# kcleal/pywfa

Measured on AMD Instinct MI355X. Metric: pairwise alignments/sec, higher is better.
Workload: dtype int16x2 offsets (reads <= 512 bp), int32 results; 1 GPU; C2: 10000000 x 150bp pairs/GPU, 2% error, gap-affine 0/4/6/2, end-to-end, scope=score, 2-bit reads resident in HBM; pairs_per_gpu=10000000, read_length=150, parallelism=pairs sharded over 1 GPU(s), no collective

## Files before the change

### pywfa_amd/csrc/host_core.hpp

```cpp
#pragma once
#include <hip/hip_runtime.h>
#include <stdarg.h>
#include <stddef.h>
#include <stdint.h>
#include <stdio.h>
#include <stdlib.h>
#include <string.h>
#include <limits.h>
#include <sched.h>
#include <string>
#include <map>
#include <unordered_map>
#include <vector>
#include <algorithm>
#include <thread>
#include <memory>
#include <atomic>

#include "wfa_hip.h"
#include "wfa_common.hpp"
#include "wfa_band.hpp"

namespace wfa { struct WfaPieceDesc; }

#pragma GCC visibility push(hidden)

extern thread_local std::string g_error;

#define WFA_COUNTER_WORDS 256
#define WFA_KNOBS(F)                                                                                              \
  F(ARENA_KB) F(BAND_DEBUG) F(BAND_SLIM) F(BAND_LDS_MAX) F(BAND_NO_WIN) F(BAND_SPLIT_MIN) F(NO_TINY_INLINE) F(BILEVEL) F(BILEVEL_WIDE_LEVELS) F(BILEVEL_PER_CU) F(BILEVEL_I32) F(BILEVEL_QCAP) F(BILEVEL_LEVELS) F(BILEVEL_LDS) F(BILEVEL_NO_1024) F(BILEVEL_HUGE_MIN) F(BILEVEL_LDS_W) F(BILEVEL_NO_SEQL) F(LANE_DYN) F(LANE_DYN_WAVES) F(BAND_LEFTOVER_WAVES_PER_CU) F(BAND_NCH) F(BAND_NO_LDS) F(BAND_NO_SPLIT) F(BAND_PB) F(PIPE_TAIL) F(LEN16) F(MAILBOX) F(MAILBOX_IDLE_US) F(TILE32)     \
  F(BAND_RECORDS) F(BAND_SPLIT_ROUNDS) F(BAND_WAVES_PER_CU) F(NO_BAND) F(NO_FAST) F(NO_SEGFULL) F(SEGFULL_PAIRS)     \
  F(SEGFULL_STAGES) F(STAGE_TIMING) F(LANE_HEUR32) F(THREADS) F(TINY_BATCH) F(WAVES_PER_CU) F(FAST_WAVES_PER_CU) F(TIMING)          \
  F(LANE_FULL) F(LANE_FULL_SPLIT) F(LANE_HEUR) F(SEG_HEUR) F(LANE_LDS_PAD_KB) F(LANE_MIN_PAIRS) F(PIPE_CHUNK) F(PIPE_THREADS) F(PACK_THREADS) F(NO_TINY_BAND) F(NO_TINY_POLL) F(UP_STREAMS) F(NO_DUAL) F(NO_WIDE) F(WIDE_ADAPT) F(WIDE_GROWS) F(WIDE_LDS_KB) F(WIDE_THREADS) F(TILE) F(TILE_T) F(TILE_WT) F(TILE_THREADS) F(TILE_PER_CU) F(NO_PIPE) F(HOST_PACK) F(GENERAL_PB) F(LANE_WAVES_PER_CU) F(LANE_REFILL_MIN) F(LANE_WINFIN) F(LANE_DEBUG) F(NO_TINY) F(PILOT_PCT) F(WIDE_ADAPT_LDS) F(LANE_NARROW_WAVES) F(PILOT_NARROW_PCT) F(CROSS_BAND) F(CROSS_TOPK_CHUNK) F(REDUCE_TIMING)
enum WfaKnob {
#define WFA_KNOB_ENUM(n) K_##n,
  WFA_KNOBS(WFA_KNOB_ENUM)
#undef WFA_KNOB_ENUM
  K_COUNT
};
struct WfaKnobs {
  int value[K_COUNT];
  bool set[K_COUNT];
  std::string fast_stages;
  void load() {
    static const char* const names[K_COUNT] = {
#define WFA_KNOB_NAME(n) "WFA_HIP_" #n,
        WFA_KNOBS(WFA_KNOB_NAME)
#undef WFA_KNOB_NAME
// ... 81 lines not shown
  std::vector<wfa::WfaPieceDesc> h_pieces;
  uint32_t* d_len16 = nullptr;
  wfa::WfaPieceDesc* d_pieces = nullptr;
  int max_width = 0;
  int max_len = 0;
  int64_t packed_bytes = 0;
  int64_t ops_bytes = 0;
  uint8_t* d_bytes = nullptr;
  int64_t* d_pboff = nullptr;
  int64_t* d_tboff = nullptr;
  WfaPairMeta* d_meta = nullptr;
  uint32_t* d_words = nullptr;
  uint8_t* d_flags = nullptr;
  int32_t* d_score = nullptr;
  int32_t* d_status = nullptr;
  uint8_t* d_ops = nullptr;
  int64_t* d_cigar_off = nullptr;
  int64_t* d_cigar_begin = nullptr;
  int32_t* d_cigar_len = nullptr;
  uint32_t* d_list_packed = nullptr;
  uint32_t* d_list_bytes = nullptr;
  uint32_t n_packed = 0, n_bytes = 0;
  uint32_t* d_fb_list2[2] = {nullptr, nullptr};
  const uint32_t* leftover_count = nullptr;
  uint32_t* d_ovf_list[2] = {nullptr, nullptr};
  uint32_t* d_counters = nullptr;
  std::vector<hipEvent_t> ev;
  size_t ev_used = 0;
  int runs_pending = 0;
  double ms_sum = 0.0; int ms_runs = 0;
// ... 122 lines not shown
```

### pywfa_amd/csrc/wfa_common.hpp

```cpp
#pragma once
#include "wfa_rtc_compat.hpp"

#define WFA_OFFSET_NULL (-1073741824)

#define WFA_INTERNAL_FALLBACK  (-1000)
#define WFA_INTERNAL_OVERFLOW  (-1001)

struct WfaPairMeta {
  uint32_t p_woff;
  uint32_t t_woff;
  int32_t plen;
  int32_t tlen;
};

struct WfaDevConfig {
  int32_t metric;
  int32_t match;
  int32_t x, o1, e1, o2, e2;
  int32_t scope;
  int32_t endsfree;
  int32_t pbf, pef, tbf, tef;
  int32_t heuristic;
  int32_t min_wf_len, max_dist_thr, steps_between, xdrop;
  int32_t max_steps;
// ... 53 lines not shown
  int g;
  int32_t* hist;
  long long hist_stride;
  int4* end_state;
  uint32_t work_begin;
  uint2* codes;
  int codes_cap;
  int ef, pbf, pef, tbf, tef;
  int heur, min_wf_len, max_dist_thr, steps_between;
  int max_steps;
  int xdrop;
  uint32_t* dyn_next;
  uint32_t dyn_chunk;
  int lin;
  int scope;
};

template <int W>
__device__ __forceinline__ int seg_from_below(int v) {
  if (W <= 16) {
    int r = __builtin_amdgcn_update_dpp(WFA_OFFSET_NULL, v, 0x111 , 0xf, 0xf, false);
    if (W == 8 && (threadIdx.x & 7) == 0) r = WFA_OFFSET_NULL;
    return r;
  }
  int r = __builtin_amdgcn_update_dpp(WFA_OFFSET_NULL, v, 0x138 , 0xf, 0xf, false);
  if (W == 32 && (threadIdx.x & 31) == 0) r = WFA_OFFSET_NULL;
  return r;
}
template <int W>
__device__ __forceinline__ int seg_from_above(int v) {
  if (W <= 16) {
// ... 13 lines not shown
```

### pywfa_amd/csrc/wfa_hip.hip

```cpp
#include <hip/hip_runtime.h>
#include <stdint.h>
#include <stdio.h>
#include <stdlib.h>
#include <string.h>
#include <limits.h>
#include <string>
#include <map>
#include <unordered_map>
#include <vector>
#include <algorithm>
#include <chrono>
#include <thread>
#include <memory>
#include <atomic>
#include <mutex>
#include <functional>
#include <ctype.h>
#include <pthread.h>
#include <sched.h>
#include <unistd.h>
#include <sys/syscall.h>

#include "host_core.hpp"
#include "wfa_pack.hpp"
// ... 306 lines not shown
  return WFA_HIP_OK;
}

extern "C" const char* wfa_hip_last_error(const wfa_hip_aligner_t* al) { return al ? al->err.c_str() : g_error.c_str(); }

wfa_hip_batch* batch_new(wfa_hip_aligner* al) {
  wfa_hip_batch* b = new wfa_hip_batch();
  b->al = al;
  al->live_batches += 1;
  return b;
}

void batch_free(wfa_hip_batch* b) {
  if (!b) return;
  (void)hipSetDevice(b->al->device);
  void* ptrs[] = {b->d_bytes, b->d_pboff, b->d_tboff, b->d_meta, b->d_words, b->d_flags, b->d_score, b->d_status,
                  b->d_ops, b->d_cigar_off, b->d_cigar_begin, b->d_cigar_len, b->d_list_packed, b->d_list_bytes,
                  b->d_fb_list2[0], b->d_fb_list2[1], b->d_ovf_list[0], b->d_ovf_list[1], b->d_counters,
                  b->d_plen, b->d_tlen, b->d_run_count, b->d_locs, b->d_run_off, b->d_len16, b->d_pieces};
  const bool timing = b->al->knobs.set[K_TIMING];
  const double t0 = timing ? std::chrono::duration<double, std::milli>(std::chrono::steady_clock::now().time_since_epoch()).count() : 0.0;
  if (b->ran && !b->synced && b->last_stream) (void)hipStreamSynchronize(b->last_stream);
  (void)hipStreamSynchronize(b->al->stream);
  const double t1 = timing ? std::chrono::duration<double, std::milli>(std::chrono::steady_clock::now().time_since_epoch()).count() : 0.0;
  for (void* p : ptrs) pool_release(b->al, p);
  for (hipEvent_t e : b->ev) (void)hipEventDestroy(e);
  if (b->upload_event) (void)hipEventDestroy(b->upload_event);
  const double t2 = timing ? std::chrono::duration<double, std::milli>(std::chrono::steady_clock::now().time_since_epoch()).count() : 0.0;
  wfa_hip_aligner* al = b->al;
  delete b;
  if (timing) fprintf(stderr, "[wfa_hip] batch_free: sync %.3f ms, release %.3f ms, host free %.3f ms\n", t1 - t0, t2 - t1,
// ... 326 lines not shown
  return WFA_HIP_OK;
}

bool wildcard_in_acgt(int wc) {
  return wc == 'A' || wc == 'C' || wc == 'G' || wc == 'T' || wc == 'a' || wc == 'c' || wc == 'g' || wc == 't';
}

int batch_alloc_common(wfa_hip_aligner* al, wfa_hip_batch* b, uint64_t total_words, int zero_tail) {
  const int64_t n = b->n;
  const size_t nn = (size_t)std::max<int64_t>(n, 1);
  HIP_TRY(al, pool_alloc(al, (void**)&b->d_meta, nn * sizeof(WfaPairMeta)));
  HIP_TRY(al, pool_alloc(al, (void**)&b->d_words, (size_t)total_words * sizeof(uint32_t)));
  HIP_TRY(al, pool_alloc(al, (void**)&b->d_flags, nn));
  HIP_TRY(al, pool_alloc(al, (void**)&b->d_score, nn * sizeof(int32_t)));
  HIP_TRY(al, pool_alloc(al, (void**)&b->d_status, nn * sizeof(int32_t)));
  HIP_TRY(al, pool_alloc(al, (void**)&b->d_fb_list2[0], nn * sizeof(uint32_t)));
  HIP_TRY(al, pool_alloc(al, (void**)&b->d_fb_list2[1], nn * sizeof(uint32_t)));
  HIP_TRY(al, pool_alloc(al, (void**)&b->d_counters, WFA_COUNTER_WORDS * sizeof(uint32_t)));
  HIP_TRY(al, hipMemsetAsync(b->d_counters, 0, WFA_COUNTER_WORDS * sizeof(uint32_t), al->stream));
  HIP_TRY(al, hipMemsetAsync(b->d_flags, 0, nn, al->stream));
  HIP_TRY(al, hipMemsetAsync(b->d_words + (total_words - (uint64_t)zero_tail), 0, (size_t)zero_tail * sizeof(uint32_t), al->stream));
  if (b->cfg.scope == WFA_SCOPE_FULL) {
    HIP_TRY(al, pool_alloc(al, (void**)&b->d_ops, (size_t)std::max<int64_t>(b->ops_bytes, 1)));
    HIP_TRY(al, pool_alloc(al, (void**)&b->d_cigar_off, ((size_t)n + 1) * sizeof(int64_t)));
    HIP_TRY(al, pool_alloc(al, (void**)&b->d_cigar_begin, nn * sizeof(int64_t)));
    HIP_TRY(al, pool_alloc(al, (void**)&b->d_cigar_len, nn * sizeof(int32_t)));
    HIP_TRY(al, pool_alloc(al, (void**)&b->d_ovf_list[0], nn * sizeof(uint32_t)));
    HIP_TRY(al, pool_alloc(al, (void**)&b->d_ovf_list[1], nn * sizeof(uint32_t)));
    HIP_TRY(al, hipMemcpyAsync(b->d_cigar_off, b->h_coff.data(), ((size_t)n + 1) * sizeof(int64_t), hipMemcpyHostToDevice, al->stream));
  }
// ... 1430 lines not shown
  if (!stages_env && b->stage_pick != 0 && c.in_count == nullptr) {
    stages = (b->stage_pick == 16) ? (b->narrow_pick == 1 ? "0189" : "189") : (b->stage_pick == 32) ? "89" : "9";
  }
  int variants[6] = {-1, -1, -1, -1, -1, -1};
  int nv = 0;
  for (const char* c = stages; *c && nv < 6; ++c) {
    const int v = *c - '0';
    if (v < 0 || v > 9) continue;
    if (v <= 1) {
      if (p.shape == WFA_SHAPE_RTC && (v == 0 || !p.lane_shape_fits)) continue;
    }
    variants[nv++] = v;
  }
  if (nv == 0) variants[nv++] = 6;
  int lane_passes = 0;
  for (int pass = 0; pass < nv; ++pass) {
    uint32_t* out_list = c.out_list(b);
    uint32_t* out_count = c.next_count(b);
    StageTimer timer(al, stream);
    int lrc;
    if (variants[pass] <= 1) {
      const bool narrow = variants[pass] == 0;
      const int lane_k = lane_passes++;
      uint32_t lane_dyn = (c.in_n >= 65536u && lane_k < 2) ? (uint32_t)std::max(0, knob(al, K_LANE_DYN, 192)) : 0u;
      const int dyn_waves = narrow ? knob(al, K_LANE_NARROW_WAVES, 24) : knob(al, K_LANE_DYN_WAVES, 16);
      if (lane_dyn && c.in_count != nullptr) {
        const int64_t expect = (b->narrow_permille >= 0 && variants[0] == 0) ? (int64_t)c.in_n * b->narrow_permille / 1000 : 0;
        const int64_t per_wave = expect / std::max<int64_t>(1, (int64_t)al->cu_count * dyn_waves * 2);
        lane_dyn = (uint32_t)std::max<int64_t>(64, std::min<int64_t>(lane_dyn, per_wave));
      }
      lrc = wfa::launch_lane(p.shape, p.sh, al->cu_count,
                             lane_dyn ? dyn_waves : knob(al, K_LANE_WAVES_PER_CU, 48),
                             wfa::lane_refill_arg(knob(al, K_LANE_REFILL_MIN, 8), knob(al, K_LANE_WINFIN, 1) != 0), b->max_len, stream, b->d_words, b->d_meta,
                             c.in_list, c.in_count, c.in_n, b->d_score, b->d_status, out_list, out_count,
                             (knob(al, K_LANE_DEBUG, 0) && al->ws) ? al->ws : nullptr, knob(al, K_LANE_LDS_PAD_KB, 0), knob(al, K_LANE_MIN_PAIRS, 0),
                             b->d_counters + (lane_k == 0 ? CNT_LANE_DYN0 : CNT_LANE_DYN1), lane_dyn, narrow ? 4 : 8);
      if (knob(al, K_LANE_DEBUG, 0) && al->ws) {
        unsigned long long c[10] = {0, 0, 0, 0, 0, 0, 0, 0, 0, 0};
        hipStreamSynchronize(stream); hipMemcpy(c, al->ws, sizeof(c), hipMemcpyDeviceToHost); hipMemset(al->ws, 0, sizeof(c));
        fprintf(stderr, "[wfa_hip] lane kernel: %llu wave-steps, %llu refills, %llu parked runs, %llu parked rounds, %llu probe blocks, %llu second-run rounds, "
                        "%llu hand-over blocks, %llu second runs, %llu entries, %llu entry rounds\n", c[0], c[1], c[2], c[3], c[4], c[5], c[6], c[7], c[8], c[9]);
      }
    } else {
      lrc = wfa::launch_seg(b->dcfg, al->cu_count, knob(al, K_FAST_WAVES_PER_CU, 256), stream, b->d_words, b->d_meta, c.in_list, c.in_count,
                            c.in_n, b->d_score, b->d_status, out_list, out_count, variants[pass]);
    }
    if (lrc != 0) { al->err = "fast kernel launch failed"; return WFA_HIP_EDEVICE; }
    if (timer.on) {
      uint32_t handed = 0;
      const float ms = timer.stop(out_count, &handed);
      fprintf(stderr, "[wfa_hip] stage %d (variant %d): %.3f ms, handed on %u pairs\n", pass, variants[pass], ms, handed);
    }
    c.advance(b, out_list, out_count);
  }
  return WFA_HIP_OK;
}

static int run_laneh_stage(wfa_hip_aligner* al, wfa_hip_batch* b, hipStream_t stream, const CascadePlan& p, Chain& c) {
  uint32_t* out_list = c.out_list(b);
  uint32_t* out_count = c.next_count(b);
// ... 1077 lines not shown
```

### pywfa_amd/csrc/wfa_lane.hpp

```cpp
#pragma once
#include "wfa_rtc_compat.hpp"
#include "wfa_common.hpp"
#include "wfa_hip.h"
#ifndef __HIPCC_RTC__
#include "wfa_rtc.hpp"
#include "wfa_shapes.hpp"
#endif

namespace wfa {

typedef short lane_s2 __attribute__((ext_vector_type(2)));
typedef unsigned short lane_u2 __attribute__((ext_vector_type(2)));

#define WFA_LANE_NULL16 (-16384)
#define WFA_LANE_NULL2 0xC000C000u
#ifndef WFA_LANE_DEBUG_COUNTERS
#define WFA_LANE_DEBUG_COUNTERS 0
#endif
#ifndef WFA_LANE_REGION_MARKS
#define WFA_LANE_REGION_MARKS 0
#endif
#if WFA_LANE_REGION_MARKS
#define WFA_LANE_MARK(name) asm volatile("; WFA_MARK " name ::: "memory")
#else
// ... 58 lines not shown
wfa_lane_kernel(const FastArgs a, const int slot_words_seq, const int refill_arg) {
  static_assert(!(FULL && HEUR), "the general form is score only");
  static_assert(NRP == 8 || (HEUR && NRP == 16) || (NRP == 4 && !FULL && !HEUR && LIN == 0),
                "the wider band exists in the general form only, the narrow one in the plain score-only form only");
  const int refill_min = refill_arg & 0xff;
  constexpr int NR = NRP, W = 2 * NR, H = NR;
  constexpr int DM = (X > OE) ? X : OE;
  constexpr int NEVER = 0x7fffffff;
  constexpr bool ENTRY = !FULL && !HEUR && LIN == 0;
  constexpr int K = ENTRY ? OE : 0, NCH = (OE + X - 1) / X;
  constexpr bool WINCH = ENTRY && NCH <= 2;
  constexpr uint32_t LNM = WINCH ? 0x3ffu : 0xffffu;
  constexpr int MH = (2 * OE) / X;
  static_assert(NCH - 1 <= MH && MH * X <= 2 * OE, "the chain's own end cells lie within the Hamming bound");
  const int mh = (refill_arg & 0x100) ? MH : NCH - 1;
  constexpr int NREC = LaneFull<OE, E>::NREC;
  extern __shared__ uint32_t lds[];
  const int slot_words = slot_words_seq;
  const int lane = threadIdx.x;
  uint32_t nwork = __builtin_amdgcn_readfirstlane(a.nwork_dev ? *a.nwork_dev : a.nwork);
  const bool dyn = !FULL && a.dyn_next != nullptr;
  bool exhausted = !dyn;
  uint32_t begin, end;
  auto grab = [&](uint32_t& b_, uint32_t& e_) -> bool {
    uint32_t nb = 0;
    if (lane == 0) nb = atomicAdd(a.dyn_next, a.dyn_chunk);
    nb = __builtin_amdgcn_readfirstlane(nb);
    if (nb >= nwork) return false;
    b_ = nb; e_ = (uint32_t)min((unsigned long long)nwork, (unsigned long long)nb + a.dyn_chunk);
    return true;
  };
  if (dyn) {
    if (!grab(begin, end)) return;
  } else {
    const uint32_t per = __builtin_amdgcn_readfirstlane((nwork + gridDim.x - 1) / gridDim.x);
    const unsigned long long begin64 = (unsigned long long)blockIdx.x * per;
    if (begin64 >= nwork) return;
    begin = (uint32_t)begin64;
    end = (uint32_t)min((unsigned long long)nwork, begin64 + per);
  }

  uint32_t pid0, pw0, ln0, pid1, pw1, ln1;
  __shared__ short wch[(WINCH && NCH == 2) ? 128 : 1];
  auto window_chain = [&](uint32_t wb, uint32_t& pid, uint32_t& pw, uint32_t& ln) -> uint32_t {
    WFA_LANE_MARK("entry_begin");
    WFA_LANE_COUNT(8);
    const int pl = (int)(ln & 0xffffu), tl = (int)(ln >> 16);
    const int nwp = (pl + 15) >> 4, ntot = nwp + ((tl + 15) >> 4), ak = tl - pl, L = min(pl, tl);
    const bool inw = (unsigned long long)wb + lane < end;
    const bool elig = inw && !(ln == 0xffffffffu || ntot + 1 > slot_words_seq || ak < 1 - 2 * H || ak > 2 * H - 1);
    bool act = elig;
    bool hact = elig && ak == 0, hend = false;
    int hm = 0;
    const uint32_t* pp = a.words + pw;
    int ch[NCH];
#pragma unroll
    for (int c = 0; c < NCH; ++c) ch[c] = WFA_LANE_NULL16;
    int ci = 0;
    const int imax = slot_words_seq >> 1;
    int base = 0;
#pragma nounroll
    for (int i = 0; i < imax && __any(act || hact); i += 2) {
      WFA_LANE_MARK("entryround_begin");
      WFA_LANE_COUNT(9);
      uint32_t x0 = 0u, x1 = 0u;
      const bool on = act || hact;
      if (on && base < L) x0 = pp[0] ^ pp[nwp];
      if (on && base + 16 < L) x1 = pp[1] ^ pp[nwp + 1];
      const int nb = L - base;
      const uint32_t k0 = nb >= 16 ? 0x55555555u : nb > 0 ? (0x55555555u >> (32 - 2 * nb)) : 0u;
      const uint32_t k1 = nb >= 32 ? 0x55555555u : nb > 16 ? (0x55555555u >> (64 - 2 * nb)) : 0u;
      unsigned long long d = (unsigned long long)((x0 | (x0 >> 1)) & k0) | ((unsigned long long)((x1 | (x1 >> 1)) & k1) << 32);
// ... 11 lines not shown
      const bool last = base + 32 >= L;
      const bool endc = act && last;
#pragma unroll
      for (int k = 0; k < NCH; ++k) ch[k] = (endc && ci == k) ? L : ch[k];
      act = act && !endc;
      hend = hend || (hact && last);
      hact = hact && !last && hm <= mh;
      pp += 2; base += 32;
      WFA_LANE_MARK("entryround_end");
    }
    const bool fin = hend && hm <= mh;
    if (fin) {
      a.score[pid] = -__mul24(hm * X, a.g);
      a.status[pid] = 0;
    }
    const uint32_t c0 = (uint32_t)ch[0];
    uint32_t lnc = elig ? (ln | ((c0 & 0x3fu) << 10) | ((c0 >> 6) << 26)) : ln;
    const bool keep = inw && !fin;
    const unsigned long long km = __ballot(keep);
    int dst = lane;
    if (__ballot(fin)) {
      const int rk = (int)__builtin_amdgcn_mbcnt_hi((uint32_t)(km >> 32), __builtin_amdgcn_mbcnt_lo((uint32_t)km, 0u));
      dst = keep ? rk : (int)__builtin_popcountll(km) + lane - rk;
      pid = (uint32_t)__builtin_amdgcn_ds_permute(dst << 2, (int)pid);
      pw = (uint32_t)__builtin_amdgcn_ds_permute(dst << 2, (int)pw);
      lnc = (uint32_t)__builtin_amdgcn_ds_permute(dst << 2, (int)lnc);
    }
    if constexpr (NCH == 2) wch[64 + dst] = (short)ch[1];
    ln = lnc;
    WFA_LANE_MARK("entry_end");
    return (uint32_t)__builtin_popcountll(km);
  };
  auto load_window = [&](uint32_t wb, uint32_t& pid, uint32_t& pw, uint32_t& ln) {
    const unsigned long long idx = (unsigned long long)wb + lane;
    pid = 0u; pw = 0u; ln = 0u;
    if (idx < end) {
      pid = a.worklist ? a.worklist[a.work_begin + idx] : (uint32_t)(a.work_begin + idx);
      const WfaPairMeta m = a.meta[pid];
      pw = m.p_woff;
      ln = (m.plen > WFA_FAST_MAX_LEN || m.tlen > WFA_FAST_MAX_LEN) ? 0xffffffffu : ((uint32_t)m.plen | ((uint32_t)m.tlen << 16));
    }
  };
  uint32_t wbase = begin, next_i = begin;
  uint32_t wn0 = 0u, wp0 = 0u, wn1 = 0u, wnext = begin;
  bool wmeta = false;
  auto slice_done = [&]() -> bool {
    if constexpr (WINCH) return wp0 >= wn0 && wn1 == 0u && wnext >= end;
    else return next_i >= end;
  };
  if constexpr (!WINCH) {
    load_window(wbase, pid0, pw0, ln0);
    load_window(wbase + 64u, pid1, pw1, ln1);
  } else {
    pid0 = pw0 = ln0 = pid1 = pw1 = ln1 = 0u;
  }

// ... 38 lines not shown
    WFA_LANE_MARK("looptop_begin");
    const int nidle = __builtin_popcountll(idle);
    if (!exhausted && slice_done() && (nidle >= refill_min || idle == ~0ull)) {
      if (grab(begin, end)) {
        wbase = begin; next_i = begin;
        if constexpr (WINCH) { wn0 = wp0 = wn1 = 0u; wnext = begin; wmeta = false; }
        else { load_window(wbase, pid0, pw0, ln0); load_window(wbase + 64u, pid1, pw1, ln1); }
      } else exhausted = true;
    }
    if (!slice_done() && (nidle >= refill_min || idle == ~0ull)) {
      WFA_LANE_MARK("refill_begin");
      WFA_LANE_COUNT(1);
      if constexpr (WINCH) {
#pragma nounroll
        while (wn1 == 0u && wnext < end) {
          if (!wmeta) load_window(wnext, pid1, pw1, ln1);
          wmeta = false;
          wn1 = window_chain(wnext, pid1, pw1, ln1);
          wnext = (end - wnext > 64u) ? wnext + 64u : end;
          if (wp0 >= wn0) {
            pid0 = pid1; pw0 = pw1; ln0 = ln1;
            if constexpr (NCH == 2) wch[lane] = wch[64 + lane];
            wn0 = wn1; wp0 = 0u; wn1 = 0u;
          }
        }
      }
      const bool is_idle = __builtin_amdgcn_inverse_ballot_w64(idle);
      const uint32_t rank = __builtin_amdgcn_mbcnt_hi((uint32_t)(idle >> 32), __builtin_amdgcn_mbcnt_lo((uint32_t)idle, 0u));
      const uint32_t navail = WINCH ? (wn0 - wp0) + wn1 : end - next_i;
      const bool take = is_idle && rank < navail;
      const uint32_t src = WINCH ? wp0 + rank : next_i + rank - wbase;
      const bool hi_w = src >= (WINCH ? wn0 : 64u);
      const int sl = (int)((WINCH ? (hi_w ? src - wn0 : src) : src) & 63u);
// ... 142 lines not shown
              if constexpr (!WINCH) { if (fin) lim[r] = WFA_LANE_NULL2; }
            }
            if constexpr (!WINCH) { if (fin) { deadline = NEVER; jt = 0; tend = 0xffffu; } }
          }
        }
      }
      if constexpr (WINCH) {
        __builtin_amdgcn_s_waitcnt(0x0F70);
        asm volatile("" ::: "memory");
      }
      if constexpr (WINCH) {
        if (wp0 >= wn0) {
          pid0 = pid1; pw0 = pw1; ln0 = ln1;
          if constexpr (NCH == 2) wch[lane] = wch[64 + lane];
          wp0 -= wn0; wn0 = wn1; wn1 = 0u;
          if (wnext < end) { load_window(wnext, pid1, pw1, ln1); wmeta = true; }
        }
      } else if (next_i - wbase >= 64u) {
        pid0 = pid1; pw0 = pw1; ln0 = ln1; wbase += 64u;
        load_window(wbase + 64u, pid1, pw1, ln1);
      }
      WFA_LANE_MARK("refill_end");
      if (WINCH && ntake == 0u && idle == ~0ull) continue;
    } else if (idle == ~0ull && exhausted) {
      rej_flush();
      break;
    }

    int hot_j = -1, hot_x = 0, hot_left = 0;
#pragma unroll
    for (int r = 0; r < NR; ++r) {
// ... 280 lines not shown
  else if (heur) hipLaunchKernelGGL((wfa_lane_kernel<X, OE, E, false, true>), dim3(grid), dim3(64), smem, stream, a, slot_words, refill_min);
  else if (full) hipLaunchKernelGGL((wfa_lane_kernel<X, OE, E, true>), dim3(grid), dim3(64), smem, stream, a, slot_words, refill_min);
  else hipLaunchKernelGGL((wfa_lane_kernel<X, OE, E, false>), dim3(grid), dim3(64), smem, stream, a, slot_words, refill_min);
  return hipGetLastError() == hipSuccess ? 0 : -1;
}

inline bool lane_heur_config(const WfaDevConfig& c, int ncomp) {
  return ncomp == 3 && c.match == 0 && c.wildcard < 0 && (c.heuristic == 0 || c.heuristic == 1);
}

inline int lane_slot_words(int max_len) {
  const int w = 2 * ((max_len + 15) >> 4) + 1;
  return w | 1;
}

inline int lane_refill_arg(int refill_min, bool winfin) { return (refill_min & 0xff) | (winfin ? 0x100 : 0); }

inline int lane_full_records(int OE, int E) { return 2 * (OE - E) + E * 17 + 1; }
inline void lane_full_geometry(uint32_t nwork, int cu_count, int per_cu, int min_pairs, int OE, int E, long long* grid_out, int* cap_out) {
  if (min_pairs <= 0) min_pairs = 256;
  long long grid = (long long)cu_count * per_cu;
  const long long max_grid = ((long long)nwork + min_pairs - 1) / std::max(min_pairs, 64);
  if (grid > max_grid) grid = max_grid;
  if (grid < 1) grid = 1;
  const long long per = ((long long)nwork + grid - 1) / grid;
  const int nrec = lane_full_records(OE, E);
  *grid_out = grid;
  *cap_out = (int)(per * nrec / 32 + 2 * nrec + 8);
}

#define WFA_LANE_RUN_SLOT 32
// ... 17 lines not shown
  if (a.lin) shape_idx = WFA_SHAPE_RTC;
  if (nrp != 8 && nrp != 4) return -1;
  if (nrp == 4 && (shape_idx == WFA_SHAPE_RTC || full || heur)) return -1;
  if (shape_idx == WFA_SHAPE_RTC) {
    struct { FastArgs a; int slot_words; int refill_min; } args = {a, slot_words, refill_min};
    return rtc_launch("wfa_lane.hpp", lane_rtc_name(sh, full, heur, a.lin), (unsigned)grid, 64, smem, stream, &args, sizeof(args));
  }
  return with_shape_index<affine_shape_count>(shape_idx, [&](auto i) {
    return launch_lane_unit<decltype(i)::value>((unsigned)grid, smem, stream, a, slot_words, refill_min, full, heur, nrp);
  });
}

inline int launch_lane(int shape_idx, const PenaltyShape& sh, int cu_count, int per_cu, int refill_min, int max_len, hipStream_t stream, const uint32_t* words,
                       const WfaPairMeta* meta, const uint32_t* worklist, const uint32_t* nwork_dev, uint32_t nwork,
                       int32_t* score, int32_t* status, uint32_t* fb_list, uint32_t* fb_count, int32_t* debug_counters = nullptr, int lds_pad_kb = 0,
                       int min_pairs = 0, uint32_t* dyn_next = nullptr, uint32_t dyn_chunk = 0, int nrp = 8) {
  FastArgs a = FastArgs();
  a.dyn_next = dyn_chunk ? dyn_next : nullptr; a.dyn_chunk = dyn_chunk;
  a.words = words; a.meta = meta; a.worklist = worklist; a.nwork_dev = nwork_dev; a.nwork = nwork;
  a.score = score; a.status = status; a.fb_list = fb_list; a.fb_count = fb_count;
  a.g = sh.g;
  a.hist = debug_counters; a.hist_stride = 0; a.end_state = nullptr; a.work_begin = 0;
  a.ef = a.pbf = a.pef = a.tbf = a.tef = 0; a.heur = 0; a.min_wf_len = a.max_dist_thr = a.steps_between = 0; a.max_steps = INT_MAX;
  return launch_lane_args(shape_idx, sh, cu_count, per_cu, refill_min, max_len, stream, a, false, lds_pad_kb, min_pairs, 0, nrp);
}

#endif

}
```

### pywfa_amd/csrc/wfa_seg.hpp

```cpp
#pragma once
#include "wfa_rtc_compat.hpp"
#include "wfa_common.hpp"
#include "wfa_hip.h"
#ifndef __HIPCC_RTC__
#include <string>
#include "wfa_rtc.hpp"
#include "wfa_shapes.hpp"
#endif

namespace wfa {

__device__ __forceinline__ uint32_t ffbl_u32(uint32_t x) {
  uint32_t r;
  asm("v_ffbl_b32 %0, %1" : "=v"(r) : "v"(x));
  return r;
}

template <int W>
__device__ __forceinline__ int seg_min(int v) {
  static_assert(W == 8 || W == 16 || W == 32, "segments inside a 32-lane group");
  v = min(v, __builtin_amdgcn_update_dpp(v, v, 0xB1 , 0xf, 0xf, false));
  v = min(v, __builtin_amdgcn_update_dpp(v, v, 0x4E , 0xf, 0xf, false));
  v = min(v, __builtin_amdgcn_update_dpp(v, v, 0x141 , 0xf, 0xf, false));
  if (W >= 16) v = min(v, __builtin_amdgcn_update_dpp(v, v, 0x140 , 0xf, 0xf, false));
// ... 3 lines not shown
template <int W>
__device__ __forceinline__ int seg_max(int v) { return ~seg_min<W>(~v); }

template <int X, int OE, int E, int W, bool LAZY, bool FULL, bool HEUR = false, int LIN = 0>
__global__ void __launch_bounds__(64)
wfa_seg_kernel(const FastArgs a) {
  static_assert(!(LAZY && FULL), "the history of a step is stored in the step itself");
  static_assert(!HEUR || (!LAZY && !FULL && W <= 32), "the general form: score only, every cell extended in its own step");
  static_assert(!LAZY || (X >= 2 && OE >= 2), "the lazy extension needs a wavefront to be consumed two steps after it is made (M is read at lags X and OE)");
  static_assert(W == 8 || W == 16 || W == 32 || W == 64, "segment width");
  constexpr int DM = (X > OE) ? X : OE;
  constexpr int NS = 64 / W, H = W / 2, LW = (W == 64) ? 6 : (W == 32) ? 5 : (W == 16) ? 4 : 3;
  constexpr unsigned long long FIELD = (W == 64) ? ~0ull : ((1ull << (W & 63)) - 1ull);
  constexpr int SW = WFA_FAST_WORDS;
  constexpr int NEVER = 0x7fffffff;
  __shared__ uint32_t lds[NS * 2 * SW + 4];
  __shared__ uint32_t ring[2][64];
  __shared__ uint32_t fbuf[64];
  __shared__ uint32_t rpid[64];
  __shared__ int rscore[64];
  const int lane = threadIdx.x;
  const int seg = lane >> LW;
  const int l = lane & (W - 1);
  const int pbias = seg * 2 * SW * 16, tbias = pbias + SW * 16;
  int kb = pbias - (l - H);
  uint32_t nwork = __builtin_amdgcn_readfirstlane(a.nwork_dev ? *a.nwork_dev : a.nwork);
  if (FULL && a.nwork_dev) {
    const uint32_t cap = a.nwork;
    if (nwork > cap) {
      for (uint32_t i = cap + blockIdx.x * 64u + threadIdx.x; i < nwork + 63u; i += gridDim.x * 64u) {
// ... 7 lines not shown
          a.fb_list[slot + __builtin_amdgcn_mbcnt_hi((uint32_t)(bm >> 32), __builtin_amdgcn_mbcnt_lo((uint32_t)bm, 0u))] = pid;
          a.status[pid] = WFA_INTERNAL_FALLBACK;
        }
      }
      nwork = cap;
    }
  }
  const uint32_t per = __builtin_amdgcn_readfirstlane((nwork + gridDim.x - 1) / gridDim.x);
  const unsigned long long begin64 = (unsigned long long)blockIdx.x * per;
  if (begin64 >= nwork) return;
  const uint32_t begin = (uint32_t)begin64;
  const uint32_t end = (uint32_t)min((unsigned long long)nwork, begin64 + per);

  uint32_t pid0, pid1;
  WfaPairMeta m0, m1;
  auto load_window = [&](uint32_t wb, uint32_t& pid, WfaPairMeta& m) {
    const unsigned long long idx = (unsigned long long)wb + lane;
    pid = 0u; m.p_woff = 0u; m.t_woff = 0u; m.plen = 0; m.tlen = 0;
    if (idx < end) { pid = a.worklist ? a.worklist[a.work_begin + idx] : (uint32_t)(a.work_begin + idx); m = a.meta[pid]; }
  };
  uint32_t wbase = begin;
  load_window(wbase, pid0, m0);
  load_window(wbase + 64u, pid1, m1);
  auto prefetch = [&](uint32_t i, uint32_t slot) {
    if (i < end) {
      const int r = (int)(i - wbase);
      uint32_t pw; int pl, tl;
      if (r < 64) {
        pw = __builtin_amdgcn_readlane(m0.p_woff, r);
        pl = __builtin_amdgcn_readlane(m0.plen, r); tl = __builtin_amdgcn_readlane(m0.tlen, r);
      } else {
        pw = __builtin_amdgcn_readlane(m1.p_woff, r - 64);
        pl = __builtin_amdgcn_readlane(m1.plen, r - 64); tl = __builtin_amdgcn_readlane(m1.tlen, r - 64);
      }
      const int ntot = ((pl + 15) >> 4) + ((tl + 15) >> 4);
      if (lane < ntot) __builtin_amdgcn_global_load_lds(a.words + pw + lane, &ring[slot][0], 4, 0, 0);
    }
  };
// ... 38 lines not shown
  int last_nonnull = 0, unreach_t = NEVER;
  bool edge = false;
  uint32_t want = (1u << NS) - 1u;
  uint32_t busy = 0;
  int gstep = 0;
  unsigned long long mcur = 0ull, mold = 0ull;

  while (true) {
    if (want) {
      do {
        const int s = __builtin_ctz(want);
        want &= want - 1u;
        if (next_i < end) {
          const uint32_t i = next_i++;
          const int r = (int)(i - wbase);
          int pl, tl; uint32_t pid;
          if (r < 64) {
            pl = __builtin_amdgcn_readlane(m0.plen, r); tl = __builtin_amdgcn_readlane(m0.tlen, r);
            pid = __builtin_amdgcn_readlane(pid0, r);
          } else {
            pl = __builtin_amdgcn_readlane(m1.plen, r - 64); tl = __builtin_amdgcn_readlane(m1.tlen, r - 64);
            pid = __builtin_amdgcn_readlane(pid1, r - 64);
          }
          const int pbf_ = (HEUR && a.ef) ? a.pbf : 0, tbf_ = (HEUR && a.ef) ? a.tbf : 0;
          const int dlo = min(-pbf_, tl - pl), dhi = max(tbf_, tl - pl);
          const bool bad = pl > WFA_FAST_MAX_LEN || tl > WFA_FAST_MAX_LEN ||
                           (HEUR ? (dhi - dlo > W - 3 || pbf_ > pl || tbf_ > tl) : (tl - pl < 1 - 2 * H || tl - pl > 2 * H - 1));
          const int akk = bad ? 0x7fff : tl - pl;
          const int c = bad ? 0 : (HEUR ? ((dlo + dhi + 1) >> 1) : ((tl - pl + 1) >> 1));
          const int nwp = (pl + 15) >> 4, ntot = nwp + ((tl + 15) >> 4);
          if (i + 1u < end) __builtin_amdgcn_s_waitcnt(0xF71);
          else __builtin_amdgcn_s_waitcnt(0xF70);
          uint32_t w = ring[par][lane];
          asm volatile("" : "+v"(w));
          if (!bad && lane < ntot) lds[s * 2 * SW + lane + ((lane >= nwp) ? SW - nwp : 0)] = w;
          prefetch(i + 2u, par);
          par ^= 1u;
          if (seg == s) {
            const int k = l - H + c;
            kb = pbias - k;
            target = (k == akk) ? tl : NEVER;
            lim = min(tl, pl + k);
            spair = pid; s0 = gstep;
            deadline = bad ? gstep - 1
                           : HEUR ? gstep + 4 * (pl + tl) + 64
                           : gstep + min(2 * (OE - E) + E * (2 * c + 2 * H - akk), 2 * (OE - E) + E * (2 * H + 2 - 2 * c + akk)) + (LAZY ? 1 : 0)
                                   - (FULL ? 1 : 0);
            if (FULL) { tslot = i; hp = reinterpret_cast<uint8_t*>(a.hist + (long long)i * a.hist_stride) + (k & (W - 1)); code = 0; }
            cur = (bad || k != 0) ? WFA_OFFSET_NULL : 0;
            if (HEUR) {
              if (!bad && a.ef && k >= -pbf_ && k <= tbf_) cur = max(k, 0);
              if (a.ef) target = bad ? NEVER : min(max(tl, pl + k - a.pef), max(pl + k, tl - a.tef));
              hdl = max(tl, pl + k); hjt = akk - (c - H); hdinit = max(pl, tl); steps_wait = a.steps_between; edge = false; have_max_sw = false;
              last_nonnull = 0; unreach_t = NEVER;
            }
#pragma unroll
            for (int d = 0; d < DM; ++d) Mh[d] = WFA_OFFSET_NULL;
#pragma unroll
            for (int d = 0; d < E; ++d) { Ih[d] = WFA_OFFSET_NULL; Dh[d] = WFA_OFFSET_NULL; }
          }
          if (LAZY) {
            const unsigned long long sm = FIELD << (s * W);
            mold &= ~sm;
            mcur = (mcur & ~sm) | (bad ? 0ull : (1ull << (s * W + H - c)));
          }
          busy |= 1u << s;
        }
      } while (want);
      if (!busy) break;
    }
    if (!LAZY) {
      int left = (cur >= 0) ? lim - cur : 0;
      if (__any(left > 0)) {
        int h = max(cur, 0) + tbias, v = max(cur + kb, pbias);
        bool more;
        do {
          const int pi = v >> 4, ti = h >> 4;
          const uint32_t p0 = lds[pi], p1 = lds[pi + 1], p2 = lds[pi + 2];
          const uint32_t t0 = lds[ti], t1 = lds[ti + 1], t2 = lds[ti + 2];
// ... 159 lines not shown
      int nm = max(nd, max(mx + 1, ni));
      if (nm > lim) nm = WFA_OFFSET_NULL;
#pragma unroll
      for (int d = E - 1; d > 0; --d) { Ih[d] = Ih[d - 1]; Dh[d] = Dh[d - 1]; }
      Ih[0] = ni; Dh[0] = nd;
      cur = nm;
      if (LAZY) { mold = mcur; mcur = __ballot(nm >= 0); }
      if (HEUR) {
        const unsigned long long eb = __ballot((l == 0 || l == W - 1) && (nm & ni & nd) >= 0);
        edge = ((eb >> (seg * W)) & FIELD) != 0ull;
      }
    }
    ++gstep;
    if (next_i - wbase >= 64u) {
      pid0 = pid1; m0 = m1; wbase += 64u;
      load_window(wbase + 64u, pid1, m1);
    }
  }
  res_flush();
  fb_flush();
}

#ifndef __HIPCC_RTC__
template <int I> int launch_seg_unit(int w, bool lazy, unsigned grid, hipStream_t stream, const FastArgs& a);
template <int I> int launch_seg_full_unit(int w, unsigned grid, hipStream_t stream, const FastArgs& a);
template <int I> int launch_seg_heur_unit(unsigned grid, hipStream_t stream, const FastArgs& a);

inline int seg_shape(const WfaDevConfig& c, PenaltyShape* sh) {
  *sh = penalty_shape(c, false);
  const int i = builtin_shape(*sh);
  if (i >= 0 && !(c.rtc && rtc_force_all())) return i;
// ... 83 lines not shown
inline void seg_full_slot(const WfaDevConfig& c, int w, int max_len, long long* code_ints, long long* event_ints, long long* slot_ints);
inline int seg_full_records(const WfaDevConfig& c, int w) {
  PenaltyShape sh;
  if (seg_shape(c, &sh) < 0) return 0;
  return 2 * (sh.OE - sh.E) + sh.E * (w + 1) + 3;
}

inline void seg_full_slot(const WfaDevConfig& c, int w, int max_len, long long* code_ints, long long* event_ints, long long* slot_ints) {
  *code_ints = (((long long)seg_full_records(c, w) * w + 15) & ~15ll) / 4;
  *event_ints = ((2ll * max_len + 16 + 15) & ~15ll) / 4;
  *slot_ints = (*code_ints + *event_ints + 2ll * max_len + 8 + 15) & ~15ll;
}

inline int launch_seg(const WfaDevConfig& c, int cu_count, int per_cu, hipStream_t stream, const uint32_t* words,
                      const WfaPairMeta* meta, const uint32_t* worklist, const uint32_t* nwork_dev, uint32_t nwork,
                      int32_t* score, int32_t* status, uint32_t* fb_list, uint32_t* fb_count, int variant) {
  FastArgs a = FastArgs();
  a.words = words; a.meta = meta; a.worklist = worklist; a.nwork_dev = nwork_dev; a.nwork = nwork;
  a.score = score; a.status = status; a.fb_list = fb_list; a.fb_count = fb_count;
  a.hist = nullptr; a.hist_stride = 0; a.end_state = nullptr; a.work_begin = 0;
  PenaltyShape sh;
  const int idx = seg_shape(c, &sh);
  if (idx < 0) return -1;
  a.g = sh.g;
  long long grid = (long long)cu_count * per_cu;
  if (!nwork_dev && grid > (long long)nwork) grid = nwork;
  if (grid < 1) grid = 1;
  const bool lazy = variant >= 6;
  const int w = (variant == 3 || variant == 7) ? 8 : (variant == 4 || variant == 8) ? 32 : (variant == 5 || variant == 9) ? 64 : 16;
  if (idx == WFA_SHAPE_RTC) return launch_seg_rtc(sh, w, lazy, false, false, (unsigned)grid, stream, a);
  return with_shape_index<affine_shape_count>(idx, [&](auto i) { return launch_seg_unit<decltype(i)::value>(w, lazy, (unsigned)grid, stream, a); });
}
// ... 5 lines not shown
```

Before: 4.369 billion alignments/s.

## Carry lane-kernel entry wavefront state into later passes to skip recomputation

The first lane pass now writes each eligible pair's early match-chain offsets, packed as two int16 values, into a new per-pair entry buffer. Later lane passes and the segmented fallback kernel read this buffer and resume the wavefront at score K instead of restarting at zero, skipping the opening steps for pairs passed on from earlier passes. This costs an extra 4-byte global store per pair and a load per retried pair, plus more complex initialisation logic in the seg kernel. That logic could be wrong in edge cases, such as equal-length pairs whose chain already reaches the end. It is enabled by default for non-full scopes and shapes with at most two chain entries.

Result: no change. 4.410 billion alignments/s (median of 6 runs) (+0.9%).

```diff
diff --git a/pywfa_amd/csrc/host_core.hpp b/pywfa_amd/csrc/host_core.hpp
--- a/pywfa_amd/csrc/host_core.hpp
+++ b/pywfa_amd/csrc/host_core.hpp
@@ -32,7 +32,7 @@
   F(ARENA_KB) F(BAND_DEBUG) F(BAND_SLIM) F(BAND_LDS_MAX) F(BAND_NO_WIN) F(BAND_SPLIT_MIN) F(NO_TINY_INLINE) F(BILEVEL) F(BILEVEL_WIDE_LEVELS) F(BILEVEL_PER_CU) F(BILEVEL_I32) F(BILEVEL_QCAP) F(BILEVEL_LEVELS) F(BILEVEL_LDS) F(BILEVEL_NO_1024) F(BILEVEL_HUGE_MIN) F(BILEVEL_LDS_W) F(BILEVEL_NO_SEQL) F(LANE_DYN) F(LANE_DYN_WAVES) F(BAND_LEFTOVER_WAVES_PER_CU) F(BAND_NCH) F(BAND_NO_LDS) F(BAND_NO_SPLIT) F(BAND_PB) F(PIPE_TAIL) F(LEN16) F(MAILBOX) F(MAILBOX_IDLE_US) F(TILE32)     \
   F(BAND_RECORDS) F(BAND_SPLIT_ROUNDS) F(BAND_WAVES_PER_CU) F(NO_BAND) F(NO_FAST) F(NO_SEGFULL) F(SEGFULL_PAIRS)     \
   F(SEGFULL_STAGES) F(STAGE_TIMING) F(LANE_HEUR32) F(THREADS) F(TINY_BATCH) F(WAVES_PER_CU) F(FAST_WAVES_PER_CU) F(TIMING)          \
-  F(LANE_FULL) F(LANE_FULL_SPLIT) F(LANE_HEUR) F(SEG_HEUR) F(LANE_LDS_PAD_KB) F(LANE_MIN_PAIRS) F(PIPE_CHUNK) F(PIPE_THREADS) F(PACK_THREADS) F(NO_TINY_BAND) F(NO_TINY_POLL) F(UP_STREAMS) F(NO_DUAL) F(NO_WIDE) F(WIDE_ADAPT) F(WIDE_GROWS) F(WIDE_LDS_KB) F(WIDE_THREADS) F(TILE) F(TILE_T) F(TILE_WT) F(TILE_THREADS) F(TILE_PER_CU) F(NO_PIPE) F(HOST_PACK) F(GENERAL_PB) F(LANE_WAVES_PER_CU) F(LANE_REFILL_MIN) F(LANE_WINFIN) F(LANE_DEBUG) F(NO_TINY) F(PILOT_PCT) F(WIDE_ADAPT_LDS) F(LANE_NARROW_WAVES) F(PILOT_NARROW_PCT) F(CROSS_BAND) F(CROSS_TOPK_CHUNK) F(REDUCE_TIMING)
+  F(LANE_FULL) F(LANE_FULL_SPLIT) F(LANE_HEUR) F(SEG_HEUR) F(LANE_LDS_PAD_KB) F(LANE_MIN_PAIRS) F(PIPE_CHUNK) F(PIPE_THREADS) F(PACK_THREADS) F(NO_TINY_BAND) F(NO_TINY_POLL) F(UP_STREAMS) F(NO_DUAL) F(NO_WIDE) F(WIDE_ADAPT) F(WIDE_GROWS) F(WIDE_LDS_KB) F(WIDE_THREADS) F(TILE) F(TILE_T) F(TILE_WT) F(TILE_THREADS) F(TILE_PER_CU) F(NO_PIPE) F(HOST_PACK) F(GENERAL_PB) F(LANE_WAVES_PER_CU) F(LANE_REFILL_MIN) F(LANE_WINFIN) F(ENTRY_CARRY) F(LANE_DEBUG) F(NO_TINY) F(PILOT_PCT) F(WIDE_ADAPT_LDS) F(LANE_NARROW_WAVES) F(PILOT_NARROW_PCT) F(CROSS_BAND) F(CROSS_TOPK_CHUNK) F(REDUCE_TIMING)
 enum WfaKnob {
 #define WFA_KNOB_ENUM(n) K_##n,
   WFA_KNOBS(WFA_KNOB_ENUM)
@@ -144,6 +144,7 @@
   uint8_t* d_flags = nullptr;
   int32_t* d_score = nullptr;
   int32_t* d_status = nullptr;
+  uint32_t* d_entry = nullptr;
   uint8_t* d_ops = nullptr;
   int64_t* d_cigar_off = nullptr;
   int64_t* d_cigar_begin = nullptr;
diff --git a/pywfa_amd/csrc/wfa_common.hpp b/pywfa_amd/csrc/wfa_common.hpp
--- a/pywfa_amd/csrc/wfa_common.hpp
+++ b/pywfa_amd/csrc/wfa_common.hpp
@@ -91,7 +91,11 @@
   uint32_t dyn_chunk;
   int lin;
   int scope;
+  uint32_t* entry;
+  int entry_in;
 };
+
+#define WFA_ENTRY_NONE 0xffffffffu
 
 template <int W>
 __device__ __forceinline__ int seg_from_below(int v) {
diff --git a/pywfa_amd/csrc/wfa_hip.hip b/pywfa_amd/csrc/wfa_hip.hip
--- a/pywfa_amd/csrc/wfa_hip.hip
+++ b/pywfa_amd/csrc/wfa_hip.hip
@@ -344,7 +344,7 @@
 void batch_free(wfa_hip_batch* b) {
   if (!b) return;
   (void)hipSetDevice(b->al->device);
-  void* ptrs[] = {b->d_bytes, b->d_pboff, b->d_tboff, b->d_meta, b->d_words, b->d_flags, b->d_score, b->d_status,
+  void* ptrs[] = {b->d_bytes, b->d_pboff, b->d_tboff, b->d_meta, b->d_words, b->d_flags, b->d_score, b->d_status, b->d_entry,
                   b->d_ops, b->d_cigar_off, b->d_cigar_begin, b->d_cigar_len, b->d_list_packed, b->d_list_bytes,
                   b->d_fb_list2[0], b->d_fb_list2[1], b->d_ovf_list[0], b->d_ovf_list[1], b->d_counters,
                   b->d_plen, b->d_tlen, b->d_run_count, b->d_locs, b->d_run_off, b->d_len16, b->d_pieces};
@@ -701,6 +701,7 @@
   HIP_TRY(al, pool_alloc(al, (void**)&b->d_flags, nn));
   HIP_TRY(al, pool_alloc(al, (void**)&b->d_score, nn * sizeof(int32_t)));
   HIP_TRY(al, pool_alloc(al, (void**)&b->d_status, nn * sizeof(int32_t)));
+  if (b->cfg.scope != WFA_SCOPE_FULL && knob(al, K_ENTRY_CARRY, 1) != 0) HIP_TRY(al, pool_alloc(al, (void**)&b->d_entry, nn * sizeof(uint32_t)));
   HIP_TRY(al, pool_alloc(al, (void**)&b->d_fb_list2[0], nn * sizeof(uint32_t)));
   HIP_TRY(al, pool_alloc(al, (void**)&b->d_fb_list2[1], nn * sizeof(uint32_t)));
   HIP_TRY(al, pool_alloc(al, (void**)&b->d_counters, WFA_COUNTER_WORDS * sizeof(uint32_t)));
@@ -2161,6 +2162,8 @@
   }
   if (nv == 0) variants[nv++] = 6;
   int lane_passes = 0;
+  uint32_t* const entry = (b->d_entry && wfa::entry_carry_shape(p.sh)) ? b->d_entry : nullptr;
+  bool entry_valid = false;
   for (int pass = 0; pass < nv; ++pass) {
     uint32_t* out_list = c.out_list(b);
     uint32_t* out_count = c.next_count(b);
@@ -2178,10 +2181,11 @@
       }
       lrc = wfa::launch_lane(p.shape, p.sh, al->cu_count,
                              lane_dyn ? dyn_waves : knob(al, K_LANE_WAVES_PER_CU, 48),
-                             wfa::lane_refill_arg(knob(al, K_LANE_REFILL_MIN, 8), knob(al, K_LANE_WINFIN, 1) != 0), b->max_len, stream, b->d_words, b->d_meta,
+                             wfa::lane_refill_arg(knob(al, K_LANE_REFILL_MIN, 8), knob(al, K_LANE_WINFIN, 1) != 0, entry_valid), b->max_len, stream, b->d_words, b->d_meta,
                              c.in_list, c.in_count, c.in_n, b->d_score, b->d_status, out_list, out_count,
                              (knob(al, K_LANE_DEBUG, 0) && al->ws) ? al->ws : nullptr, knob(al, K_LANE_LDS_PAD_KB, 0), knob(al, K_LANE_MIN_PAIRS, 0),
-                             b->d_counters + (lane_k == 0 ? CNT_LANE_DYN0 : CNT_LANE_DYN1), lane_dyn, narrow ? 4 : 8);
+                             b->d_counters + (lane_k == 0 ? CNT_LANE_DYN0 : CNT_LANE_DYN1), lane_dyn, narrow ? 4 : 8, entry);
+      entry_valid = entry != nullptr;
       if (knob(al, K_LANE_DEBUG, 0) && al->ws) {
         unsigned long long c[10] = {0, 0, 0, 0, 0, 0, 0, 0, 0, 0};
         hipStreamSynchronize(stream); hipMemcpy(c, al->ws, sizeof(c), hipMemcpyDeviceToHost); hipMemset(al->ws, 0, sizeof(c));
@@ -2190,7 +2194,7 @@
       }
     } else {
       lrc = wfa::launch_seg(b->dcfg, al->cu_count, knob(al, K_FAST_WAVES_PER_CU, 256), stream, b->d_words, b->d_meta, c.in_list, c.in_count,
-                            c.in_n, b->d_score, b->d_status, out_list, out_count, variants[pass]);
+                            c.in_n, b->d_score, b->d_status, out_list, out_count, variants[pass], entry_valid ? entry : nullptr);
     }
     if (lrc != 0) { al->err = "fast kernel launch failed"; return WFA_HIP_EDEVICE; }
     if (timer.on) {
diff --git a/pywfa_amd/csrc/wfa_lane.hpp b/pywfa_amd/csrc/wfa_lane.hpp
--- a/pywfa_amd/csrc/wfa_lane.hpp
+++ b/pywfa_amd/csrc/wfa_lane.hpp
@@ -96,6 +96,8 @@
   constexpr int MH = (2 * OE) / X;
   static_assert(NCH - 1 <= MH && MH * X <= 2 * OE, "the chain's own end cells lie within the Hamming bound");
   const int mh = (refill_arg & 0x100) ? MH : NCH - 1;
+  constexpr bool CARRY_IN = WINCH && NRP == 8;
+  const bool carry_in = CARRY_IN && (refill_arg & 0x200) != 0 && a.entry != nullptr;
   constexpr int NREC = LaneFull<OE, E>::NREC;
   extern __shared__ uint32_t lds[];
   const int slot_words = slot_words_seq;
@@ -123,21 +125,29 @@
   }
 
   uint32_t pid0, pw0, ln0, pid1, pw1, ln1;
+  uint32_t en1 = WFA_ENTRY_NONE;
   __shared__ short wch[(WINCH && NCH == 2) ? 128 : 1];
-  auto window_chain = [&](uint32_t wb, uint32_t& pid, uint32_t& pw, uint32_t& ln) -> uint32_t {
+  auto window_chain = [&](uint32_t wb, uint32_t& pid, uint32_t& pw, uint32_t& ln, const uint32_t en) -> uint32_t {
     WFA_LANE_MARK("entry_begin");
     WFA_LANE_COUNT(8);
     const int pl = (int)(ln & 0xffffu), tl = (int)(ln >> 16);
     const int nwp = (pl + 15) >> 4, ntot = nwp + ((tl + 15) >> 4), ak = tl - pl, L = min(pl, tl);
     const bool inw = (unsigned long long)wb + lane < end;
     const bool elig = inw && !(ln == 0xffffffffu || ntot + 1 > slot_words_seq || ak < 1 - 2 * H || ak > 2 * H - 1);
-    bool act = elig;
-    bool hact = elig && ak == 0, hend = false;
+    const bool carried = CARRY_IN && elig && en != WFA_ENTRY_NONE;
+    bool act = elig && !carried;
+    bool hact = elig && ak == 0 && !carried, hend = false;
     int hm = 0;
     const uint32_t* pp = a.words + pw;
     int ch[NCH];
 #pragma unroll
     for (int c = 0; c < NCH; ++c) ch[c] = WFA_LANE_NULL16;
+    if constexpr (CARRY_IN) {
+      if (carried) {
+        ch[0] = (int)(short)(en & 0xffffu);
+        if constexpr (NCH == 2) ch[1] = (int)(short)(en >> 16);
+      }
+    }
     int ci = 0;
     const int imax = slot_words_seq >> 1;
     int base = 0;
@@ -179,6 +189,8 @@
       a.score[pid] = -__mul24(hm * X, a.g);
       a.status[pid] = 0;
     }
+    if (a.entry != nullptr && inw && !carried)
+      a.entry[pid] = elig ? (((uint32_t)ch[0] & 0xffffu) | ((uint32_t)(NCH == 2 ? ch[NCH - 1] : WFA_LANE_NULL16) << 16)) : WFA_ENTRY_NONE;
     const uint32_t c0 = (uint32_t)ch[0];
     uint32_t lnc = elig ? (ln | ((c0 & 0x3fu) << 10) | ((c0 >> 6) << 26)) : ln;
     const bool keep = inw && !fin;
@@ -205,6 +217,9 @@
       pw = m.p_woff;
       ln = (m.plen > WFA_FAST_MAX_LEN || m.tlen > WFA_FAST_MAX_LEN) ? 0xffffffffu : ((uint32_t)m.plen | ((uint32_t)m.tlen << 16));
     }
+  };
+  auto load_entry = [&](uint32_t wb, uint32_t pid) -> uint32_t {
+    return (carry_in && (unsigned long long)wb + lane < end) ? a.entry[pid] : WFA_ENTRY_NONE;
   };
   uint32_t wbase = begin, next_i = begin;
   uint32_t wn0 = 0u, wp0 = 0u, wn1 = 0u, wnext = begin;
@@ -273,9 +288,12 @@
       if constexpr (WINCH) {
 #pragma nounroll
         while (wn1 == 0u && wnext < end) {
-          if (!wmeta) load_window(wnext, pid1, pw1, ln1);
+          if (!wmeta) {
+            load_window(wnext, pid1, pw1, ln1);
+            if constexpr (CARRY_IN) en1 = load_entry(wnext, pid1);
+          }
           wmeta = false;
-          wn1 = window_chain(wnext, pid1, pw1, ln1);
+          wn1 = window_chain(wnext, pid1, pw1, ln1, en1);
           wnext = (end - wnext > 64u) ? wnext + 64u : end;
           if (wp0 >= wn0) {
             pid0 = pid1; pw0 = pw1; ln0 = ln1;
@@ -448,7 +466,10 @@
           pid0 = pid1; pw0 = pw1; ln0 = ln1;
           if constexpr (NCH == 2) wch[lane] = wch[64 + lane];
           wp0 -= wn0; wn0 = wn1; wn1 = 0u;
-          if (wnext < end) { load_window(wnext, pid1, pw1, ln1); wmeta = true; }
+          if (wnext < end) {
+            load_window(wnext, pid1, pw1, ln1); wmeta = true;
+            if constexpr (CARRY_IN) en1 = load_entry(wnext, pid1);
+          }
         }
       } else if (next_i - wbase >= 64u) {
         pid0 = pid1; pw0 = pw1; ln0 = ln1; wbase += 64u;
@@ -759,7 +780,9 @@
   return w | 1;
 }
 
-inline int lane_refill_arg(int refill_min, bool winfin) { return (refill_min & 0xff) | (winfin ? 0x100 : 0); }
+inline int lane_refill_arg(int refill_min, bool winfin, bool entry_in = false) { return (refill_min & 0xff) | (winfin ? 0x100 : 0) | (entry_in ? 0x200 : 0); }
+
+inline bool entry_carry_shape(const PenaltyShape& sh) { return (sh.OE + sh.X - 1) / sh.X <= 2; }
 
 inline int lane_full_records(int OE, int E) { return 2 * (OE - E) + E * 17 + 1; }
 inline void lane_full_geometry(uint32_t nwork, int cu_count, int per_cu, int min_pairs, int OE, int E, long long* grid_out, int* cap_out) {
@@ -807,8 +830,9 @@
 inline int launch_lane(int shape_idx, const PenaltyShape& sh, int cu_count, int per_cu, int refill_min, int max_len, hipStream_t stream, const uint32_t* words,
                        const WfaPairMeta* meta, const uint32_t* worklist, const uint32_t* nwork_dev, uint32_t nwork,
                        int32_t* score, int32_t* status, uint32_t* fb_list, uint32_t* fb_count, int32_t* debug_counters = nullptr, int lds_pad_kb = 0,
-                       int min_pairs = 0, uint32_t* dyn_next = nullptr, uint32_t dyn_chunk = 0, int nrp = 8) {
+                       int min_pairs = 0, uint32_t* dyn_next = nullptr, uint32_t dyn_chunk = 0, int nrp = 8, uint32_t* entry = nullptr) {
   FastArgs a = FastArgs();
+  a.entry = entry;
   a.dyn_next = dyn_chunk ? dyn_next : nullptr; a.dyn_chunk = dyn_chunk;
   a.words = words; a.meta = meta; a.worklist = worklist; a.nwork_dev = nwork_dev; a.nwork = nwork;
   a.score = score; a.status = status; a.fb_list = fb_list; a.fb_count = fb_count;
diff --git a/pywfa_amd/csrc/wfa_seg.hpp b/pywfa_amd/csrc/wfa_seg.hpp
--- a/pywfa_amd/csrc/wfa_seg.hpp
+++ b/pywfa_amd/csrc/wfa_seg.hpp
@@ -41,6 +41,10 @@
   constexpr unsigned long long FIELD = (W == 64) ? ~0ull : ((1ull << (W & 63)) - 1ull);
   constexpr int SW = WFA_FAST_WORDS;
   constexpr int NEVER = 0x7fffffff;
+  constexpr int NCH = (OE + X - 1) / X;
+  constexpr bool ENTRY = !FULL && !HEUR && LIN == 0 && W >= 16 && NCH <= 2;
+  constexpr int K = OE;
+  const bool entry_in = ENTRY && a.entry_in != 0 && a.entry != nullptr;
   __shared__ uint32_t lds[NS * 2 * SW + 4];
   __shared__ uint32_t ring[2][64];
   __shared__ uint32_t fbuf[64];
@@ -78,14 +82,19 @@
 
   uint32_t pid0, pid1;
   WfaPairMeta m0, m1;
-  auto load_window = [&](uint32_t wb, uint32_t& pid, WfaPairMeta& m) {
+  uint32_t en0 = WFA_ENTRY_NONE, en1 = WFA_ENTRY_NONE;
+  auto load_window = [&](uint32_t wb, uint32_t& pid, WfaPairMeta& m, uint32_t& en) {
     const unsigned long long idx = (unsigned long long)wb + lane;
     pid = 0u; m.p_woff = 0u; m.t_woff = 0u; m.plen = 0; m.tlen = 0;
-    if (idx < end) { pid = a.worklist ? a.worklist[a.work_begin + idx] : (uint32_t)(a.work_begin + idx); m = a.meta[pid]; }
+    if (ENTRY) en = WFA_ENTRY_NONE;
+    if (idx < end) {
+      pid = a.worklist ? a.worklist[a.work_begin + idx] : (uint32_t)(a.work_begin + idx); m = a.meta[pid];
+      if (ENTRY) { if (entry_in) en = a.entry[pid]; }
+    }
   };
   uint32_t wbase = begin;
-  load_window(wbase, pid0, m0);
-  load_window(wbase + 64u, pid1, m1);
+  load_window(wbase, pid0, m0, en0);
+  load_window(wbase + 64u, pid1, m1, en1);
   auto prefetch = [&](uint32_t i, uint32_t slot) {
     if (i < end) {
       const int r = (int)(i - wbase);
@@ -154,13 +163,15 @@
         if (next_i < end) {
           const uint32_t i = next_i++;
           const int r = (int)(i - wbase);
-          int pl, tl; uint32_t pid;
+          int pl, tl; uint32_t pid, en = WFA_ENTRY_NONE;
           if (r < 64) {
             pl = __builtin_amdgcn_readlane(m0.plen, r); tl = __builtin_amdgcn_readlane(m0.tlen, r);
             pid = __builtin_amdgcn_readlane(pid0, r);
+            if (ENTRY) en = __builtin_amdgcn_readlane(en0, r);
           } else {
             pl = __builtin_amdgcn_readlane(m1.plen, r - 64); tl = __builtin_amdgcn_readlane(m1.tlen, r - 64);
             pid = __builtin_amdgcn_readlane(pid1, r - 64);
+            if (ENTRY) en = __builtin_amdgcn_readlane(en1, r - 64);
           }
           const int pbf_ = (HEUR && a.ef) ? a.pbf : 0, tbf_ = (HEUR && a.ef) ? a.tbf : 0;
           const int dlo = min(-pbf_, tl - pl), dhi = max(tbf_, tl - pl);
@@ -176,15 +187,18 @@
           if (!bad && lane < ntot) lds[s * 2 * SW + lane + ((lane >= nwp) ? SW - nwp : 0)] = w;
           prefetch(i + 2u, par);
           par ^= 1u;
+          const int ec0 = (int)(short)(en & 0xffffu), ec1 = (int)(short)(en >> 16);
+          const bool ent = ENTRY && en != WFA_ENTRY_NONE && !bad && ec0 >= 0 && !(tl == pl && (ec0 == tl || ec1 == tl));
+          const int sk = ent ? K : 0;
           if (seg == s) {
             const int k = l - H + c;
             kb = pbias - k;
             target = (k == akk) ? tl : NEVER;
             lim = min(tl, pl + k);
-            spair = pid; s0 = gstep;
+            spair = pid; s0 = gstep - sk;
             deadline = bad ? gstep - 1
                            : HEUR ? gstep + 4 * (pl + tl) + 64
-                           : gstep + min(2 * (OE - E) + E * (2 * c + 2 * H - akk), 2 * (OE - E) + E * (2 * H + 2 - 2 * c + akk)) + (LAZY ? 1 : 0)
+                           : s0 + min(2 * (OE - E) + E * (2 * c + 2 * H - akk), 2 * (OE - E) + E * (2 * H + 2 - 2 * c + akk)) + (LAZY ? 1 : 0)
                                    - (FULL ? 1 : 0);
             if (FULL) { tslot = i; hp = reinterpret_cast<uint8_t*>(a.hist + (long long)i * a.hist_stride) + (k & (W - 1)); code = 0; }
             cur = (bad || k != 0) ? WFA_OFFSET_NULL : 0;
@@ -198,11 +212,30 @@
             for (int d = 0; d < DM; ++d) Mh[d] = WFA_OFFSET_NULL;
 #pragma unroll
             for (int d = 0; d < E; ++d) { Ih[d] = WFA_OFFSET_NULL; Dh[d] = WFA_OFFSET_NULL; }
+            if constexpr (ENTRY) {
+              if (ent) {
+                const int ch[2] = {ec0, (ec1 >= 0) ? ec1 : WFA_OFFSET_NULL};
+#pragma unroll
+                for (int d = 0; d < DM; ++d) {
+                  const int sc = K - 1 - d;
+                  if (sc >= 0 && sc % X == 0) Mh[d] = (k == 0) ? ch[sc / X] : WFA_OFFSET_NULL;
+                }
+                Ih[0] = (k == 1) ? ec0 + 1 : WFA_OFFSET_NULL;
+                Dh[0] = (k == -1) ? ec0 : WFA_OFFSET_NULL;
+                int nm = max(Ih[0], Dh[0]);
+                if (K % X == 0) nm = max(nm, (k == 0) ? ch[NCH - 1] + 1 : WFA_OFFSET_NULL);
+                cur = (nm > lim) ? WFA_OFFSET_NULL : nm;
+              }
+            }
           }
           if (LAZY) {
             const unsigned long long sm = FIELD << (s * W);
             mold &= ~sm;
-            mcur = (mcur & ~sm) | (bad ? 0ull : (1ull << (s * W + H - c)));
+            if constexpr (ENTRY) {
+              mcur = (mcur & ~sm) | (__ballot(seg == s && cur >= 0) & sm);
+            } else {
+              mcur = (mcur & ~sm) | (bad ? 0ull : (1ull << (s * W + H - c)));
+            }
           }
           busy |= 1u << s;
         }
@@ -392,7 +425,8 @@
     ++gstep;
     if (next_i - wbase >= 64u) {
       pid0 = pid1; m0 = m1; wbase += 64u;
-      load_window(wbase + 64u, pid1, m1);
+      if (ENTRY) en0 = en1;
+      load_window(wbase + 64u, pid1, m1, en1);
     }
   }
   res_flush();
@@ -506,8 +540,10 @@
 
 inline int launch_seg(const WfaDevConfig& c, int cu_count, int per_cu, hipStream_t stream, const uint32_t* words,
                       const WfaPairMeta* meta, const uint32_t* worklist, const uint32_t* nwork_dev, uint32_t nwork,
-                      int32_t* score, int32_t* status, uint32_t* fb_list, uint32_t* fb_count, int variant) {
+                      int32_t* score, int32_t* status, uint32_t* fb_list, uint32_t* fb_count, int variant,
+                      const uint32_t* entry = nullptr) {
   FastArgs a = FastArgs();
+  a.entry = const_cast<uint32_t*>(entry); a.entry_in = entry != nullptr;
   a.words = words; a.meta = meta; a.worklist = worklist; a.nwork_dev = nwork_dev; a.nwork = nwork;
   a.score = score; a.status = status; a.fb_list = fb_list; a.fb_count = fb_count;
   a.hist = nullptr; a.hist_stride = 0; a.end_state = nullptr; a.work_begin = 0;
```
